# Brian-Acosta/fcc_qp

Measured on NVIDIA B200. Metric: qps_solved_per_sec_batch_65536_cold, higher is better.
Workload: dtype f64

## Files before the change

### fcc_qp_b200/csrc/fccqp_capi.cu

```cuda
#include <cuda_runtime.h>

#include <atomic>
#include <chrono>
#include <cmath>
#include <cstdarg>
#include <cstdio>
#include <cstring>
#include <map>
#include <memory>
#include <mutex>
#include <thread>
#include <string>
#include <vector>

#include "../../include/fccqp.h"
#include "fccqp_kernel.cuh"
#include "fccqp_struct.cuh"
#include "fccqp_warp.cuh"
#include "fccqp_polish.cuh"

namespace {

thread_local std::string g_err;
std::atomic<long long> g_launches{0};
// ... 91 lines not shown
using KernelFn = void (*)(const fccqp::SolveParams);

struct DevSwitches {
  bool no_warp = false;
  bool no_shared = false;
  int full_inverse_at = 0;
  int cta_cap = 0;
#ifdef FCCQP_DEV
  bool profile = false;
#endif
};

const DevSwitches& dev_switches() {
  static const DevSwitches s = [] {
    DevSwitches d;
    d.no_warp = getenv("FCCQP_NO_WARP") != nullptr;
    d.no_shared = getenv("FCCQP_NO_SHARED") != nullptr;
    if (const char* v = getenv("FCCQP_FULL_INVERSE_AT")) d.full_inverse_at = atoi(v) < 1 ? 1 : atoi(v);
    if (const char* v = getenv("FCCQP_CTAS_PER_SM")) d.cta_cap = atoi(v);
#ifdef FCCQP_DEV
    d.profile = getenv("FCCQP_PROFILE") != nullptr;
#endif
    return d;
  }();
  return s;
}

int check_shape(const DeviceCtx& ctx, int n, int m, int nc) {
  const int N = n + m;
  if (N < 1) return fail(FCCQP_E_INVALID, "n + m must be >= 1");
  const fccqp::Layout l(n, m, nc);
  if (l.N8 > 256 || l.bytes() > (size_t)ctx.max_smem_optin)
    return fail(FCCQP_E_UNSUPPORTED,
                "n + m = %d (padded %d) needs %zu B of shared memory per QP (limit %d B, 256 rows): too large "
                "for the shared-memory-resident kernels", N, l.N8, l.bytes(), ctx.max_smem_optin);
  return FCCQP_OK;
}

template <int kThreads, int kMinBlocks>
KernelFn solve_instance(bool shared, bool f32, bool adapt) {
  using fccqp::fccqp_solve_kernel;
  if (shared) return fccqp_solve_kernel<kThreads, kMinBlocks, true, false>;
  if (f32) return adapt ? fccqp_solve_kernel<kThreads, kMinBlocks, false, true, true> : fccqp_solve_kernel<kThreads, kMinBlocks, false, true>;
  return adapt ? fccqp_solve_kernel<kThreads, kMinBlocks, false, false, true> : fccqp_solve_kernel<kThreads, kMinBlocks, false, false>;
}
KernelFn pick_kernel(int threads, bool shared, bool f32, bool adapt) {
  return threads == 128 ? solve_instance<128, 4>(shared, f32, adapt) : solve_instance<256, 2>(shared, f32, adapt);
}

template <int kThreads, int kMinBlocks>
KernelFn struct_instance(bool adapt) {
  return adapt ? fccqp::fccqp_struct_kernel<kThreads, kMinBlocks, true> : fccqp::fccqp_struct_kernel<kThreads, kMinBlocks, false>;
}

bool host_classify(int n, int m, const double* Q, long long q_rs, long long q_cs, const double* A, long long a_rs,
                   long long a_cs, int* nr, int* ndp, int* nd0) {
  std::vector<int> rowcnt(m > 0 ? m : 1, 0), one_row(n, -1);
  std::vector<char> type(n, 0);
  bool ok = true;
  for (int j = 0; j < n; ++j) {
    bool sep = true;
    for (int i = 0; i < n && sep; ++i)
      if (i != j && (Q[i * q_rs + j * q_cs] != 0.0 || Q[j * q_rs + i * q_cs] != 0.0)) sep = false;
    const double qd = Q[j * q_rs + j * q_cs];
    int nnz = 0, kr = 0;
    for (int k = 0; k < m; ++k) if (A[k * a_rs + j * a_cs] != 0.0) { ++nnz; kr = k; }
    if (!sep || !(qd >= 0.0)) type[j] = fccqp::VT_R;
    else if (qd < 1e-200) { type[j] = fccqp::VT_D0; if (nnz == 0) ok = false; }
    else if (nnz <= 1) { type[j] = fccqp::VT_D1; if (nnz == 1) { one_row[j] = kr; ++rowcnt[kr]; } }
    else type[j] = fccqp::VT_DP;
  }
  *nr = *ndp = *nd0 = 0;
  for (int j = 0; j < n; ++j) {
    if (type[j] == fccqp::VT_D1 && one_row[j] >= 0 && rowcnt[one_row[j]] > 1) type[j] = fccqp::VT_DP;
    if (type[j] == fccqp::VT_R) ++*nr; else if (type[j] == fccqp::VT_DP) ++*ndp; else if (type[j] == fccqp::VT_D0) ++*nd0;
  }
  return ok;
}

int geometry(DeviceCtx& ctx, KernelFn fn, int threads, size_t smem, int B, int qps_per_cta, LaunchInfo* li) {
  int c = 0;
  {
    std::lock_guard<std::mutex> lk(ctx.mu);
    const auto key = std::make_pair((const void*)fn, smem);
    auto it = ctx.occupancy.find(key);
    if (it != ctx.occupancy.end()) c = it->second;
    else {
      CUDA_TRY(cudaFuncSetAttribute(fn, cudaFuncAttributeMaxDynamicSharedMemorySize, ctx.max_smem_optin));
      CUDA_TRY(cudaOccupancyMaxActiveBlocksPerMultiprocessor(&c, fn, threads, smem));
      if (c < 1) return fail(FCCQP_E_UNSUPPORTED, "kernel does not fit on an SM (smem %zu B)", smem);
      ctx.occupancy[key] = c;
    }
  }
  const int cap = dev_switches().cta_cap;
  if (cap > 0 && cap < c) c = cap;
  const int need = (B + qps_per_cta - 1) / qps_per_cta;
  *li = {c * ctx.num_sms < need ? c * ctx.num_sms : need, threads, (int)smem, c};
  return FCCQP_OK;
}

struct Scratch {
  static constexpr size_t kWork = 0;
  static constexpr size_t kWork2 = 1;
  static constexpr size_t kListCount = 2;
  static constexpr size_t kProbe = 4;
  static constexpr size_t kLpt = 8;
  static constexpr size_t kHeader = 16;
  unsigned int* w = nullptr;
  size_t B = 0;
  int* list() const { return reinterpret_cast<int*>(w + kHeader); }
  int* order() const { return reinterpret_cast<int*>(w + kHeader + B); }
};

int begin_call(fccqp::SolveParams& p, cudaStream_t stream, bool lpt_hint, long long slots, Scratch* s) {
  const bool lpt = lpt_hint && p.n_iter != nullptr && p.B >= 2 * slots;
  s->B = (size_t)p.B;
  CUDA_TRY(cudaMallocAsync(&s->w, (Scratch::kHeader + (lpt ? 2 : 1) * s->B) * sizeof(unsigned int), stream));
  CUDA_TRY(cudaMemsetAsync(s->w, 0, Scratch::kHeader * sizeof(unsigned int), stream));
  p.work_counter = s->w + Scratch::kWork;
  if (lpt) {
    fccqp::lpt_order_kernel<<<(p.B + 255) / 256, 256, 0, stream>>>(p.n_iter, p.B, p.full_inverse_at, s->order(),
                                                                   s->w + Scratch::kLpt, s->w + Scratch::kLpt + 1);
    CUDA_TRY(cudaGetLastError());
    p.index_list = s->order();
  }
  return FCCQP_OK;
}

int end_call(const Scratch& s, cudaStream_t stream, int launches, const LaunchInfo& li, const StructInfo& si) {
  CUDA_TRY(cudaFreeAsync(s.w, stream));
  g_launches.fetch_add(launches);
  std::lock_guard<std::mutex> lk(g_info_mu);
  g_last_launch = li;
  g_last_struct = si;
  return FCCQP_OK;
}

StructInfo dense_info(const DeviceCtx& ctx, int rows) {
  StructInfo si;
  si.rows = si.rows_dense = rows;
  si.device = ctx.device;
  return si;
}

#ifdef FCCQP_DEV
struct PhaseProfile {
  unsigned long long* d = nullptr;
  int start(cudaStream_t stream, fccqp::SolveParams* p) {
    if (!dev_switches().profile) return FCCQP_OK;
    CUDA_TRY(cudaMalloc(&d, 16 * sizeof(unsigned long long)));
    CUDA_TRY(cudaMemsetAsync(d, 0, 16 * sizeof(unsigned long long), stream));
    p->prof = d;
    return FCCQP_OK;
  }
  int report(cudaStream_t stream, const char* kernel, const char* const (&names)[16], int B, int grid) {
    if (!d) return FCCQP_OK;
    unsigned long long h[16];
    CUDA_TRY(cudaMemcpyAsync(h, d, sizeof(h), cudaMemcpyDeviceToHost, stream));
    CUDA_TRY(cudaStreamSynchronize(stream));
    CUDA_TRY(cudaFree(d));
    const double qps = (double)h[14];
    double tot = 0;
    for (int i = 0; i < 16; ++i) if (names[i]) tot += (double)h[i];
    fprintf(stderr, "[fccqp %s profile] B=%d grid=%d qps=%llu", kernel, B, grid, h[14]);
    if (!names[15]) fprintf(stderr, " iters=%llu", h[15]);
    fprintf(stderr, " cycles/QP=%.0f\n", qps > 0 ? tot / qps : 0.0);
    for (int i = 0; i < 16; ++i)
      if (names[i])
        fprintf(stderr, "   %-14s %10.0f cyc/QP  %5.1f%%\n", names[i], qps > 0 ? (double)h[i] / qps : 0.0,
                tot > 0 ? 100.0 * (double)h[i] / tot : 0.0);
// ... 22 lines not shown
  CUDA_TRY(cudaGetLastError());
  return end_call(s, stream, 1, li, dense_info(ctx, N));
}

int launch_shared(DeviceCtx& ctx, fccqp::SolveParams p, cudaStream_t stream, const Scratch& s) {
  const int threads = p.lay.N8 <= 128 ? 128 : 256;
  KernelFn fn = pick_kernel(threads, true, false, false);
  LaunchInfo li;
  int rc = geometry(ctx, fn, threads, p.lay.bytes(), p.B, 1, &li);
  if (rc) return rc;
  p.shared_mode = 2;
  if (!p.warm) {
    fccqp::SolveParams a = p;
    a.shared_mode = 1;
    a.pending_count = s.w + Scratch::kListCount;
    a.pending_list = s.list();
    fn<<<li.grid, li.block, li.smem, stream>>>(a);
    CUDA_TRY(cudaGetLastError());
    p.count_dev = a.pending_count;
    p.index_list = s.list();
    p.work_counter = s.w + Scratch::kWork2;
  }
  fn<<<li.grid, li.block, li.smem, stream>>>(p);
  CUDA_TRY(cudaGetLastError());
  return end_call(s, stream, p.warm ? 1 : 2, li, dense_info(ctx, p.lay.N8));
}

constexpr int kNotApplicable = 1;

int launch_struct(DeviceCtx& ctx, const fccqp::SolveParams& p, cudaStream_t stream, const Scratch& s, const StructHint& hint,
                  KernelFn general, const LaunchInfo& gli) {
  int caps[3] = {hint.caps[0], hint.caps[1], hint.caps[2]};
  if (hint.mode != FCCQP_STRUCTURE_CAPS) {
    const int ns = p.B < 128 ? p.B : 128;
    int* d_probe = reinterpret_cast<int*>(s.w + Scratch::kProbe);
    if (p.n <= 128 && p.m <= 128) fccqp::fccqp_struct_probe_kernel<128><<<ns, 128, 0, stream>>>(p, ns, d_probe);
    else fccqp::fccqp_struct_probe_kernel<256><<<ns, 256, 0, stream>>>(p, ns, d_probe);
    CUDA_TRY(cudaGetLastError());
    int h[4];
    {
      std::lock_guard<std::mutex> lk(ctx.mu);
      CUDA_TRY(cudaMemcpyAsync(ctx.h_probe, d_probe, sizeof(h), cudaMemcpyDeviceToHost, stream));
      CUDA_TRY(cudaStreamSynchronize(stream));
      memcpy(h, ctx.h_probe, sizeof(h));
    }
    g_launches.fetch_add(1);
    if (h[3] != 0) return kNotApplicable;
    caps[0] = h[0]; caps[1] = h[1]; caps[2] = h[2];
  }
  if (caps[0] < 0 || caps[0] > p.n || caps[1] < 0 || caps[2] < 0 || caps[0] + caps[1] + caps[2] > p.n) return kNotApplicable;
  const fccqp::StructLayout sl(p.n, p.m, p.nc, caps[0], caps[1] + caps[2], caps[2]);
  if (sl.N8c + 8 > p.lay.N8 || sl.bytes() > (size_t)ctx.max_smem_optin) return kNotApplicable;
  const int need = p.n > sl.N8c ? p.n : sl.N8c;
  const bool adapt = p.adapt_k > 0;
  KernelFn fn;
  int threads;
  if (need <= 64) { threads = 64; fn = struct_instance<64, 8>(adapt); }
  else if (need <= 96) { threads = 96; fn = struct_instance<96, 5>(adapt); }
  else if (need <= 128) { threads = 128; fn = struct_instance<128, 4>(adapt); }
  else { threads = 256; fn = struct_instance<256, 2>(adapt); }
  LaunchInfo li;
  int rc = geometry(ctx, fn, threads, sl.bytes(), p.B, 1, &li);
  if (rc) return rc;
  fccqp::SolveParams a = p;
  a.slay = sl;
  a.pending_count = s.w + Scratch::kListCount;
  a.pending_list = s.list();
  const long long neT = sl.n8 >> 3, NBr = sl.nr8c >> 3, mt = sl.mt;
  a.op_stride = (2 * mt * neT + neT * NBr + neT * (neT + 1) / 2) * 64 + 8 * neT;
  CUDA_TRY(cudaMallocAsync(&a.op_scratch, (size_t)li.grid * a.op_stride * sizeof(double), stream));
#ifdef FCCQP_DEV
  PhaseProfile prof;
  if ((rc = prof.start(stream, &a))) return rc;
#endif
  fn<<<li.grid, li.block, li.smem, stream>>>(a);
  CUDA_TRY(cudaGetLastError());
  CUDA_TRY(cudaFreeAsync(a.op_scratch, stream));
#ifdef FCCQP_DEV
  if ((rc = prof.report(stream, "struct", kStructPhases, p.B, li.grid))) return rc;
#endif
  fccqp::SolveParams b = p;
  b.count_dev = a.pending_count;
  b.index_list = s.list();
  b.work_counter = s.w + Scratch::kWork2;
  general<<<gli.grid, gli.block, gli.smem, stream>>>(b);
  CUDA_TRY(cudaGetLastError());
  CUDA_TRY(cudaMemcpyAsync(ctx.h_deferred, a.pending_count, sizeof(unsigned int), cudaMemcpyDeviceToHost, stream));
  StructInfo si;
  si.used = 1; si.nr = caps[0]; si.ndp = caps[1]; si.nd0 = caps[2]; si.rows = sl.N8c; si.rows_dense = p.lay.N8; si.device = ctx.device;
  return end_call(s, stream, 2, li, si);
}

int launch_general(DeviceCtx& ctx, fccqp::SolveParams p, cudaStream_t stream, const Scratch& s, KernelFn fn, const LaunchInfo& li) {
#ifdef FCCQP_DEV
  PhaseProfile prof;
  int rc = prof.start(stream, &p);
  if (rc) return rc;
#endif
  fn<<<li.grid, li.block, li.smem, stream>>>(p);
  CUDA_TRY(cudaGetLastError());
#ifdef FCCQP_DEV
  if ((rc = prof.report(stream, "general", kGeneralPhases, p.B, li.grid))) return rc;
#endif
  return end_call(s, stream, 1, li, dense_info(ctx, p.lay.N8));
}

int launch_solve(DeviceCtx& ctx, fccqp::SolveParams p, cudaStream_t stream, int precision, const StructHint& hint) {
  if (p.B == 0) return FCCQP_OK;
  int rc = check_shape(ctx, p.n, p.m, p.nc);
  if (rc) return rc;
  const DevSwitches& sw = dev_switches();
  const bool f32 = precision != FCCQP_PRECISION_FP64;
  const bool small = p.n + p.m <= 32;
  p.lay = fccqp::Layout(p.n, p.m, p.nc);
  p.full_inverse_at = sw.full_inverse_at ? sw.full_inverse_at : (small ? 8 : 6);
  p.struct_refine = hint.refine;
  if (small && (precision == FCCQP_PRECISION_FP32 || (!f32 && !sw.no_warp)))
    return launch_warp(ctx, p, stream, precision == FCCQP_PRECISION_FP32, hint.lpt);

  const int threads = p.lay.N8 <= 128 ? 128 : 256;
  KernelFn general = pick_kernel(threads, false, f32, p.adapt_k > 0);
  LaunchInfo li;
  Scratch s;
  if ((rc = geometry(ctx, general, threads, p.lay.bytes(), p.B, 1, &li)) ||
      (rc = begin_call(p, stream, hint.lpt, (long long)li.ctas_per_sm * ctx.num_sms, &s)))
    return rc;
  if (!sw.no_shared && !f32 && p.q_bs == 0 && (p.m == 0 || p.a_bs == 0) && p.B >= 4 * li.ctas_per_sm * ctx.num_sms)
    return launch_shared(ctx, p, stream, s);
  if (!f32 && hint.mode != FCCQP_STRUCTURE_DENSE && p.m > 0 &&
      (rc = launch_struct(ctx, p, stream, s, hint, general, li)) != kNotApplicable)
    return rc;
  return launch_general(ctx, p, stream, s, general, li);
}

int check_dims(int n, int m, int nc, int lcs) {
  if (n < 0 || m < 0 || nc < 0) return fail(FCCQP_E_INVALID, "negative dimension");
  if (nc % 3 != 0) return fail(FCCQP_E_INVALID, "nc = %d must be a multiple of 3 (src/fcc_qp.cpp:32)", nc);
  if (lcs < 0 || lcs + nc > n)
    return fail(FCCQP_E_INVALID, "lambda_c_start + nc = %d exceeds num_vars = %d (src/fcc_qp.cpp:33)", lcs + nc, n);
  if (n < 1) return fail(FCCQP_E_INVALID, "num_vars must be >= 1");
  return FCCQP_OK;
}

// ... 754 lines not shown
```

### fcc_qp_b200/csrc/fccqp_kernel.cuh

```cuda
#pragma once
#include <cuda_runtime.h>
#include <stdint.h>

namespace fccqp {

struct Layout {
  int n, m, nc;
  int n8, m8, N8;
  int NB, NBx;
  int NB32, NT;
  int NBT;
  int off_M, off_dinv, off_dneg, off_tbuf, off_ybuf, off_xs, off_lcbar, off_muc, off_mu;
  int off_red, off_int;
  int doubles_total;
  static inline int up2(int v) { return (v + 1) & ~1; }
  Layout() = default;
  Layout(int n_, int m_, int nc_) {
    n = n_; m = m_; nc = nc_;
    n8 = (n + 7) & ~7; m8 = (m + 7) & ~7; N8 = n8 + m8;
    NB = N8 >> 3; NBx = n8 >> 3;
    NB32 = (N8 + 31) >> 5; NT = NB32 * 32;
    NBT = NB * (NB + 1) / 2;
    int o = 0;
    off_M = o;     o += NBT * 64;
// ... 59 lines not shown
    off_muc = o;   o += up2(nc + 2);
    off_mu = o;    o += up2(nc / 3 + 2);
    off_red = o;   o += 4 * 32 + 16;
    off_int = o;
    int io = 8;
    io_vtype = io;  io += n8;
    io_vpos = io;   io += n8;
    io_rlist = io;  io += nr8c + 8;
    io_dplist = io; io += ndp8c + 8;
    io_d0list = io; io += nd08c + 8;
    io_d1var = io;  io += m8 + 8;
    io_rowcnt = io; io += m8 + 8;
    io_wtot = io;   io += 32 * 3;
    io_nzflag = io; io += n8;
    io_colcnt = io; io += n8;
    io_colk = io;   io += n8;
    ints_total = io;
    o += (io + 1) / 2;
    doubles_total = o;
  }
  size_t bytes() const { return (size_t)doubles_total * sizeof(double); }
};

struct SolveParams {
  int B, n, m, nc, lcs;
  int max_iter, warm;
  int shared_mode;
  const int* index_list;
  const unsigned int* count_dev;
  int* pending_list;
  unsigned int* pending_count;
  int full_inverse_at;
  double rho, eps_fcone, eps_bound;
  double alpha;
  int adapt_k;
  const double* Q;   long long q_bs, q_rs, q_cs;
  const double* b;   long long b_bs;
  const double* A;   long long a_bs, a_rs, a_cs;
  const double* beq; long long beq_bs;
  const double* mu;  long long mu_bs;
  const double* lb;  long long lb_bs;
  const double* ub;  long long ub_bs;
  double* x; double* mu_x; double* mu_c;
  int* n_iter; int* status;
  double* res_b; double* res_f; double* bviol; double* fviol;
  unsigned int* work_counter;
  unsigned long long* cycles;
  unsigned long long* prof;
  Layout lay;
  StructLayout slay;
  int struct_refine;
  double* op_scratch;
  long long op_stride;
};

__device__ __forceinline__ double warp_max(double v) {
#pragma unroll
  for (int o = 16; o > 0; o >>= 1) v = fmax(v, __shfl_xor_sync(0xffffffffu, v, o));
  return v;
}
__device__ __forceinline__ double warp_sum(double v) {
#pragma unroll
  for (int o = 16; o > 0; o >>= 1) v += __shfl_xor_sync(0xffffffffu, v, o);
  return v;
}

template <bool kSum>
__device__ __forceinline__ void block_reduce2(double& a, double& b, double* red, int& parity) {
  const int lane = threadIdx.x & 31, warp = threadIdx.x >> 5, nw = blockDim.x >> 5;
  double va = a, vb = b;
#pragma unroll
  for (int o = 16; o > 0; o >>= 1) {
    const double oa = __shfl_xor_sync(0xffffffffu, va, o), ob = __shfl_xor_sync(0xffffffffu, vb, o);
    if (kSum) { va += oa; vb += ob; } else { va = fmax(va, oa); vb = fmax(vb, ob); }
  }
  double* r = red + parity * 64;
  if (lane == 0) { r[warp] = va; r[32 + warp] = vb; }
  __syncthreads();
  double ra = r[0], rb = r[32];
#pragma unroll 1
  for (int w = 1; w < nw; ++w) {
    if (kSum) { ra += r[w]; rb += r[32 + w]; } else { ra = fmax(ra, r[w]); rb = fmax(rb, r[32 + w]); }
  }
  a = ra; b = rb;
  parity ^= 1;
}

constexpr double kPivotRatio = 1e-12;
constexpr double kRegDelta = 1e-10;
constexpr int kRegTries = 4;

__device__ __forceinline__ double fast_rcp(double d) {
  double x;
  asm("rcp.approx.ftz.f64 %0, %1;" : "=d"(x) : "d"(d));
  const double e = fma(-d, x, 1.0);
  const double t = fma(e, e, e);
  return fma(x, t, x);
}

__device__ __forceinline__ void cp_async4(void* smem_dst, const void* gsrc) {
  const unsigned s = (unsigned)__cvta_generic_to_shared(smem_dst);
  asm volatile("cp.async.ca.shared.global [%0], [%1], 4;" ::"r"(s), "l"(gsrc) : "memory");
}
__device__ __forceinline__ void cp_async8(double* smem_dst, const double* gsrc) {
  const unsigned s = (unsigned)__cvta_generic_to_shared(smem_dst);
  asm volatile("cp.async.ca.shared.global [%0], [%1], 8;" ::"r"(s), "l"(gsrc) : "memory");
// ... 1225 lines not shown
```

### fcc_qp_b200/csrc/fccqp_struct.cuh

```cuda
#pragma once
#include "fccqp_kernel.cuh"

namespace fccqp {

enum : int { VT_R = 0, VT_DP = 1, VT_D1 = 2, VT_D0 = 3, VT_NONE = 4 };

struct VarClass {
  int type, pos, krow, nnz;
  double aval, qd;
};

struct StructInts {
  int *vtype, *vpos, *rlist, *dplist, *d0list, *d1var, *rowcnt, *wtot, *nzflag, *colcnt, *colk;
};

__device__ __forceinline__ unsigned smem_u32(const void* p) { return (unsigned)__cvta_generic_to_shared(p); }
__device__ __forceinline__ void cp_async8_s(unsigned smem_dst, const double* gsrc) {
  asm volatile("cp.async.ca.shared.global [%0], [%1], 8;" ::"r"(smem_dst), "l"(gsrc) : "memory");
}
__device__ __forceinline__ void mbar_init(unsigned long long* bar, int count) {
  asm volatile("mbarrier.init.shared::cta.b64 [%0], %1;" ::"r"(smem_u32(bar)), "r"(count) : "memory");
  asm volatile("fence.mbarrier_init.release.cluster;" ::: "memory");
}
__device__ __forceinline__ void bulk_g2s(void* dst, const void* src, unsigned bytes, unsigned long long* bar) {
// ... 720 lines not shown
      if (ib < NBF) s0 += col_dot8(M + tile_off(ib, tb) + colo, colc, flip, tbuf + ib * 8);
      out[t] = xbt + (s0 + s1);
    }
    __syncthreads();
    rx = 0.0; rc = 0.0;
    if (is_x) {
      val = out[ci];
      const double xh = relax ? fma(alpha, val, (1.0 - alpha) * xbar) : val;
      const double xb = clampd(xh + mux, lb, ub);
      xbar = xb;
      const double rr = xh - xb;
      mux += rr;
      rx = fabs(rr);
      if (!in_cone) tbuf[ci] = shift * (xbar - mux);
    }
    if (contact) {
      double x0 = out[c0], x1 = out[c1], x2 = out[c2];
      if (relax) {
        x0 = fma(alpha, x0, (1.0 - alpha) * lcbar[3 * t]);
        x1 = fma(alpha, x1, (1.0 - alpha) * lcbar[3 * t + 1]);
        x2 = fma(alpha, x2, (1.0 - alpha) * lcbar[3 * t + 2]);
      }
      double o0, o1, o2;
      project_cone3(x0 + muc[3 * t], x1 + muc[3 * t + 1], x2 + muc[3 * t + 2], mu_t, o0, o1, o2);
      lcbar[3 * t] = o0; lcbar[3 * t + 1] = o1; lcbar[3 * t + 2] = o2;
      const double r0 = x0 - o0, r1 = x1 - o1, r2 = x2 - o2;
      const double m0 = muc[3 * t] + r0, m1 = muc[3 * t + 1] + r1, m2 = muc[3 * t + 2] + r2;
      muc[3 * t] = m0; muc[3 * t + 1] = m1; muc[3 * t + 2] = m2;
      rc = fmax(fabs(r0), fmax(fabs(r1), fabs(r2)));
      tbuf[c0] = shift * (o0 - m0); tbuf[c1] = shift * (o1 - m1); tbuf[c2] = shift * (o2 - m2);
    }
    if (rx != rx || rc != rc) nan_seen = 1;
    conv = __syncthreads_and((rc < a.eps_fcone) && (rx < a.eps_bound));
    if (conv || iter + 1 == a.iters) break;
  }
  if (is_x) smem[a.xs + t] = val;
  th.xbar = xbar; th.mux = mux; th.x = val; th.rx = rx; th.rc = rc; th.conv = conv; th.nan_seen = nan_seen;
  return iter;
}

#ifdef FCCQP_DEV
#define SPROF(slot)                                                        \
  do {                                                                     \
    if (p.prof && tid == 0) {                                              \
      const long long t_now = clock64();                                   \
      s_prof[slot] += (unsigned long long)(t_now - t_prof);                \
      t_prof = t_now;                                                      \
    }                                                                      \
  } while (0)
#else
#define SPROF(slot) do { } while (0)
#endif

template <int kThreads, int kMinBlocks, bool kAdapt>
__global__ void __launch_bounds__(kThreads, kMinBlocks) fccqp_struct_kernel(const SolveParams p) {
  extern __shared__ __align__(16) double smem[];
  const StructLayout& L = p.slay;
  const int tid = threadIdx.x, lane = tid & 31, warp = tid >> 5;
  constexpr int kWarps = kThreads / 32;
  const int n = p.n, m = p.m, nc = p.nc, lcs = p.lcs;
  const int n8 = L.n8, m8 = L.m8, mt = L.mt, dptc = L.dptc;

  double* const M = smem + L.off_M;
  double* const AP = smem + L.off_AP;
  double* const dinv = smem + L.off_dinv;
  double* const dneg = smem + L.off_dneg;
  double* const vd = smem + L.off_vd;
  double* const hinv = smem + L.off_hinv;
  double* const beqs = smem + L.off_beq;
  double* const qd_s = smem + L.off_qd;
  double* const xs = smem + L.off_xs;
  double* const lcbar = smem + L.off_lcbar;
  double* const muc = smem + L.off_muc;
  double* const vmu = smem + L.off_mu;
  double* const red = smem + L.off_red;
  int* const ibuf = reinterpret_cast<int*>(smem + L.off_int);
  int* const s_work = ibuf;
  StructInts I;
  I.vtype = ibuf + L.io_vtype; I.vpos = ibuf + L.io_vpos; I.rlist = ibuf + L.io_rlist; I.dplist = ibuf + L.io_dplist;
  I.d0list = ibuf + L.io_d0list; I.d1var = ibuf + L.io_d1var; I.rowcnt = ibuf + L.io_rowcnt; I.wtot = ibuf + L.io_wtot;
  I.nzflag = ibuf + L.io_nzflag; I.colcnt = ibuf + L.io_colcnt; I.colk = ibuf + L.io_colk;
  double* const rf = smem + L.off_rf;
  StageCtl sc;
  sc.bar = reinterpret_cast<unsigned long long*>(ibuf + 2);
  sc.phase = 0;
  if (tid == 0) mbar_init(sc.bar, 1);

#ifdef FCCQP_DEV
  unsigned long long* const s_prof = reinterpret_cast<unsigned long long*>(smem + L.off_red + 4 * 32);
  long long t_prof = 0;
  if (p.prof && tid == 0) { for (int i = 0; i < 16; ++i) s_prof[i] = 0; t_prof = clock64(); }
#endif
  int parity = 0;
  const int t = tid;
  const bool is_x = t < n;
  const bool in_cone = is_x && t >= lcs && t < lcs + nc;
  const int fr = lane >> 2, fq = lane & 3;
  const int fragC = (fr << 3) + (((fq ^ (fr >> 1)) & 3) << 1);
  const long long q_slow = p.q_cs <= p.q_rs ? p.q_rs : p.q_cs;
  const long long q_fast = p.q_cs <= p.q_rs ? p.q_cs : p.q_rs;
  const bool q_dense = q_fast == 1 && q_slow == n;
  const bool a_dense = (p.a_cs == 1 && p.a_rs == n) || (p.a_rs == 1 && p.a_cs == m);

  int w_next = 0;
  if (tid == 0) {
    w_next = (int)atomicAdd(p.work_counter, 1u);
    if (p.index_list && w_next < p.B) w_next = p.index_list[w_next];
  }
  for (;;) {
    __syncthreads();
    if (tid == 0) {
      s_work[0] = w_next;
      if (w_next < p.B) {
        w_next = (int)atomicAdd(p.work_counter, 1u);
        if (p.index_list && w_next < p.B) w_next = p.index_list[w_next];
      }
    }
    __syncthreads();
    const int qp = s_work[0];
    if (qp >= p.B) break;
    const double* Qg = p.Q + (size_t)qp * p.q_bs;
    const double* Ag = p.A + (size_t)qp * p.a_bs;
    SPROF(0);

    double v_b = 0.0, v_lb = 0.0, v_ub = 0.0, v_mux = 0.0, v_xbar = 0.0, v_x = 0.0;
    int finite_bounds = 0;
    if (is_x) {
      v_b = p.b[(size_t)qp * p.b_bs + t];
      v_lb = p.lb[(size_t)qp * p.lb_bs + t];
      v_ub = p.ub[(size_t)qp * p.ub_bs + t];
      if (p.warm) { v_x = p.x[(size_t)qp * n + t]; v_mux = p.mu_x[(size_t)qp * n + t]; }
    }
    if (t < m) beqs[t] = p.beq[(size_t)qp * p.beq_bs + t];
    if (t < nc / 3) vmu[t] = p.mu[(size_t)qp * p.mu_bs + t];
    if (t < nc) muc[t] = p.warm ? p.mu_c[(size_t)qp * nc + t] : 0.0;
    for (int e = t; e < L.ndp8c + 8; e += kThreads) { vd[e] = 0.0; hinv[e] = 0.0; }

    const long long t_start = clock64();
    unsigned long long fact_cycles = 0;
    int status_flag = 0;
    int n_iter = 0;
    double res_x = 0.0, res_c = 0.0;

    VarClass vc;
    StructQP S;
    const bool q_vec = q_fast == 1 && (n & 1) == 0 && (q_slow & 1) == 0 && (reinterpret_cast<uintptr_t>(Qg) & 15) == 0;
    const bool a_vec = p.a_cs == 1 && (n & 1) == 0 && (p.a_rs & 1) == 0 && (reinterpret_cast<uintptr_t>(Ag) & 15) == 0;
    sc.q_bulk = q_vec && q_slow == n;
    sc.a_bulk = a_vec && p.a_rs == n;
    bool defer = struct_classify<kThreads>(n, m, n8, m8, Qg, q_slow, q_fast, q_vec, Ag, p.a_rs, p.a_cs, a_vec, M, L.stage_cap, sc,
                                           qd_s, rf, I, L.nr8c, L.ndp8c, L.nd08c, vc, S.nr, S.ndp, S.nd0) != 0;
    SPROF(1);
    if (tid == 0 && w_next < p.B) {
      if (q_dense) l2_prefetch(p.Q + (size_t)w_next * p.q_bs, (size_t)n * n * sizeof(double));
      if (a_dense) l2_prefetch(p.A + (size_t)w_next * p.a_bs, (size_t)m * n * sizeof(double));
    }
    S.nr8 = (S.nr + 7) & ~7;
    const int NBr = S.nr8 >> 3;
    const int yrow = t - S.nr8;
    if (is_x && (!isinf(v_lb) || !isinf(v_ub))) finite_bounds = 1;
    if (t < n8) xs[t] = v_x;
    const bool eqc = (nc == 0) && (__syncthreads_or(finite_bounds) == 0);
    const bool presolve = eqc || !p.warm;

    for (int pass = presolve ? 0 : 1; pass < 2 && !defer; ++pass) {
      if (pass == 1 && eqc) break;
      if (pass == 1) {
        v_xbar = v_x;
        if (in_cone) lcbar[t - lcs] = v_x;
        __syncthreads();
        n_iter = p.max_iter;
      }
      const int iters = pass == 0 ? 1 : p.max_iter;
      double shift = pass == 0 ? 0.0 : p.rho;
      VarClass ve = vc;
      StructQP Se = S;
      if (pass == 1 && S.nd0 > 0) {
        if (vc.type == VT_D0) { ve.type = VT_DP; ve.pos = S.ndp + (vc.pos - S.nr8 - m8); }
        Se.ndp = S.ndp + S.nd0;
        Se.nd0 = 0;
      }
      Se.dpt = (Se.ndp + 7) >> 3;
      Se.N8 = S.nr8 + m8 + ((Se.nd0 + 7) & ~7);
      Se.NB = Se.N8 >> 3;
      Se.NB32 = (Se.N8 + 31) >> 5;
      double hi = (ve.type == VT_DP || ve.type == VT_D1) ? 1.0 / (ve.qd + shift) : 0.0;
      bool factored = false;
      bool full_inverse = false;
      bool full_op = false;
      int ci = -1, NBF = 0, NF = 0;
      double v_xbase = 0.0;

#pragma unroll 1
      for (int iter = 0; iter < iters; ++iter) {
        double val = v_x;
        if (!(pass == 1 && iter == 0 && presolve)) {
          if (!factored) {
            factored = true;
            const long long t_f0 = clock64();
            {
              const int nbt = (Se.NB * (Se.NB + 1)) >> 1;
              const double2 z2 = make_double2(0.0, 0.0);
              for (int e = t; e < nbt * 32; e += kThreads) st2(M + 2 * e, z2);
              for (int e = t; e < mt * dptc * 32; e += kThreads) st2(AP + 2 * e, z2);
            }
            if (is_x) { I.vtype[t] = ve.type; I.vpos[t] = ve.pos; }
            __syncthreads();
            {
              constexpr int kCol = kThreads / 32;
              const unsigned mS = smem_u32(M), apS = smem_u32(AP);
              int ckind[kCol], cps[kCol], chf[kCol];
              unsigned cof[kCol];
#pragma unroll
              for (int u = 0; u < kCol; ++u) {
                const int j = lane + 32 * u;
                const int ty = j < n ? I.vtype[j] : VT_NONE;
                const int ps = j < n ? I.vpos[j] : 0;
                ckind[u] = ty == VT_R ? 0 : (ty == VT_DP ? 1 : (ty == VT_D0 ? 2 : 3));
                cps[u] = ps;
                chf[u] = (ps & 7) >> 1;
                cof[u] = ty == VT_D0 ? mS + (unsigned)tile_off(ps >> 3, 0) * 8u + ((ps & 7) << 6)
                                     : (unsigned)(((ps >> 3) << 9) + ((ps & 1) << 3));
              }
#pragma unroll 1
              for (int a = warp; a < S.nr; a += kWarps) {
                const double* qrow = Qg + (long long)I.rlist[a] * q_slow;
                const unsigned rowS = mS + (unsigned)tile_off(a >> 3, 0) * 8u + ((a & 7) << 6);
                const int rh = (a & 7) >> 1;
#pragma unroll
                for (int u = 0; u < kCol; ++u)
                  if (ckind[u] == 0 && cps[u] <= a)
                    cp_async8_s(rowS + cof[u] + (((chf[u] ^ rh) & 3) << 4), qrow + (long long)(lane + 32 * u) * q_fast);
              }
              if (p.a_cs == 1 || p.a_rs != 1) {
#pragma unroll 1
                for (int k = warp; k < m; k += kWarps) {
                  const double* arow = Ag + (long long)k * p.a_rs;
                  const int yr = S.nr8 + k, rh = (k & 7) >> 1;
                  const unsigned rowM = mS + (unsigned)tile_off(yr >> 3, 0) * 8u + ((k & 7) << 6);
                  const unsigned rowP = apS + (unsigned)((k >> 3) * dptc) * 512u + ((k & 7) << 6);
                  const unsigned colT = (unsigned)(((yr >> 3) << 9) + ((yr & 1) << 3));
#pragma unroll
                  for (int u = 0; u < kCol; ++u) {
                    const int kd = ckind[u];
                    const unsigned base = kd == 0 ? rowM : (kd == 1 ? rowP : colT);
                    if (kd < 3) cp_async8_s(base + cof[u] + (((chf[u] ^ rh) & 3) << 4), arow + (long long)(lane + 32 * u) * p.a_cs);
                  }
                }
              } else {
// ... 12 lines not shown
              }
            }
            if (t < Se.N8) {
              const bool pad = (t >= S.nr && t < S.nr8) || (yrow >= m && yrow < m8) || (t >= S.nr8 + m8 + Se.nd0);
              if (pad) M[mat_off(t, t)] = 1.0;
            }
            if (ve.type == VT_D0) M[mat_off(ve.pos, ve.pos)] = ve.qd + shift;
            if (ve.type == VT_DP) hinv[ve.pos] = hi;
            SPROF(2);
            cp_async_wait_all();
            __syncthreads();
            SPROF(3);
            if (t < S.nr && shift != 0.0) M[mat_off(t, t)] += shift;
            {
              const int ntile = (mt * (mt + 1)) >> 1;
#pragma unroll 1
              for (int w = warp; w < ntile; w += kWarps) {
                int Ic = 0;
                while (((Ic + 1) * (Ic + 2)) >> 1 <= w) ++Ic;
                const int Jc = w - ((Ic * (Ic + 1)) >> 1);
                double2 ca = make_double2(0.0, 0.0), cb = make_double2(0.0, 0.0);
                const double* ai = AP + (size_t)(Ic * dptc) * 64 + fragC;
                const double* aj = AP + (size_t)(Jc * dptc) * 64 + fragC;
#pragma unroll 1
                for (int kt = 0; kt < Se.dpt; ++kt) {
                  const double2 a = ld2(ai + 64 * kt), b = ld2(aj + 64 * kt), h = ld2(hinv + 8 * kt + 2 * fq);
                  dmma(ca.x, ca.y, a.x * h.x, b.x);
                  dmma(cb.x, cb.y, a.y * h.y, b.y);
                }
                st2(M + tile_off(NBr + Ic, NBr + Jc) + fragC, make_double2(-(ca.x + cb.x), -(ca.y + cb.y)));
              }
            }
            __syncthreads();
            if (ve.type == VT_D1 && ve.nnz == 1) M[mat_off(S.nr8 + ve.krow, S.nr8 + ve.krow)] -= ve.aval * ve.aval * hi;
            if (yrow >= m && yrow < m8) M[mat_off(t, t)] = 1.0;
            __syncthreads();
            SPROF(4);
            factor_tiles<kThreads>(M, dinv, dneg, Se.NB, Se.NB32);
            SPROF(5);
            fact_cycles += (unsigned long long)(clock64() - t_f0);
            {
              bool badp = false;
              const bool neg = yrow >= 0 && yrow < m;
              const double dn = t < Se.N8 ? dneg[t] : 0.0;
              if (t < Se.N8) badp = !isfinite(dn) || (neg ? !(dn > 0.0) : !(dn < 0.0));
              double pc = neg ? fabs(dn) : 0.0, pu = 0.0;
              block_reduce2<false>(pc, pu, red, parity);
              if (neg && fabs(dn) < kPivotRatio * pc) badp = true;
              if (__syncthreads_or(badp)) { defer = true; break; }
            }
          }

          const double w = (pass == 1 && is_x) ? (in_cone ? (lcbar[t - lcs] - muc[t - lcs]) : (v_xbar - v_mux)) : 0.0;
          const bool make_op = pass == 1 && !full_inverse && iter >= p.full_inverse_at;
#pragma unroll 1
          for (int rep = make_op ? 0 : 1; rep < 2; ++rep) {
            const bool base_solve = rep == 0;
            if (!base_solve && full_op) {
              val = full_op_apply(M, smem + L.off_tbuf, smem + L.off_ybuf, smem + L.off_sred, ci, shift * w, NBF, NF);
              break;
            }
            const bool op = !base_solve && full_inverse;
            double r = 0.0;
            if (is_x) r = (base_solve || pass == 0) ? -v_b : (op ? shift * w : -(v_b - shift * w));
#ifdef FCCQP_DEV
            const double res = struct_xsolve<kThreads>(p, L, smem, I, Se, ve, Qg, Ag, q_slow, q_fast, r, hi, shift, op, op,
                                                       pass == 0 && p.struct_refine != 0, q_vec && a_vec, s_prof, t_prof);
#else
            const double res = struct_xsolve<kThreads>(p, L, smem, I, Se, ve, Qg, Ag, q_slow, q_fast, r, hi, shift, op, op,
                                                       pass == 0 && p.struct_refine != 0, q_vec && a_vec);
#endif
            if (base_solve) {
              v_xbase = res;
              __syncthreads();
              SPROF(12);
              complete_inverse<kThreads>(M, Se.NB);
              SPROF(13);
              form_g<kThreads>(M, dinv, Se.NB, Se.NB, Se.NB);
              SPROF(15);
              full_inverse = true;
              if (p.op_stride > 0) {
                FullOpDims fd;
                fd.NBr = NBr; fd.mt = mt; fd.dptc = dptc; fd.dpt = Se.dpt;
                fd.ne = n - S.nr; fd.neT = (fd.ne + 7) >> 3; fd.NBF = NBr + fd.neT; fd.NF = fd.NBF * 8;
                if (fd.NF <= kThreads && fd.NF <= L.NTc && tile_off(fd.NBF, 0) <= L.stage_cap) {
                  const bool is_d1 = is_x && ve.type == VT_D1;
                  const unsigned b1 = __ballot_sync(0xffffffffu, is_d1);
                  if (lane == 0) I.wtot[warp] = __popc(b1);
                  __syncthreads();
                  int o1 = 0;
  #pragma unroll
                  for (int w2 = 0; w2 < kWarps; ++w2) if (w2 < warp) o1 += I.wtot[w2];
                  int epos = -1;
                  if (is_x && ve.type == VT_DP) epos = ve.pos;
                  else if (is_d1) epos = Se.ndp + o1 + __popc(b1 & ((1u << lane) - 1u));
                  ci = is_x ? (ve.type == VT_R ? ve.pos : S.nr8 + epos) : -1;
                  NBF = fd.NBF; NF = fd.NF;
                  build_full_op<kThreads>(M, AP, hinv, p.op_scratch + (size_t)blockIdx.x * p.op_stride, fd, is_x ? ve.type : VT_NONE,
                                          epos, ve.krow, ve.nnz, ve.aval, hi);
                  SPROF(10);
                  double* const tb2 = smem + L.off_tbuf;
                  double* const xb2 = smem + L.off_ybuf;
                  if (t < NF) { tb2[t] = 0.0; xb2[t] = 0.0; }
                  __syncthreads();
                  if (ci >= 0) xb2[ci] = v_xbase;
                  full_op = true;
                }
              }
            } else {
              val = op ? v_xbase + res : res;
            }
          }
        }
        SPROF(12);

        if (pass == 0) {
          v_x = val;
          if (t < n8) xs[t] = is_x ? val : 0.0;
          __syncthreads();
          continue;
        }

        if (is_x) { xs[t] = val; v_x = val; }
        __syncthreads();
        double rx = 0.0, rc = 0.0, dz = 0.0;
        const bool relax = p.alpha != 1.0;
        if (is_x) {
          const double xh = relax ? fma(p.alpha, val, (1.0 - p.alpha) * v_xbar) : val;
          const double xb = clampd(xh + v_mux, v_lb, v_ub);
          if (kAdapt) dz = fabs(xb - v_xbar);
          v_xbar = xb;
          const double rr = xh - xb;
          v_mux += rr;
          rx = fabs(rr);
        }
        if (t < nc / 3) {
          const int o = lcs + 3 * t;
          double x0 = xs[o], x1 = xs[o + 1], x2 = xs[o + 2];
          if (relax) {
            x0 = fma(p.alpha, x0, (1.0 - p.alpha) * lcbar[3 * t]);
            x1 = fma(p.alpha, x1, (1.0 - p.alpha) * lcbar[3 * t + 1]);
            x2 = fma(p.alpha, x2, (1.0 - p.alpha) * lcbar[3 * t + 2]);
          }
          double o0, o1, o2;
          project_cone3(x0 + muc[3 * t], x1 + muc[3 * t + 1], x2 + muc[3 * t + 2], vmu[t], o0, o1, o2);
          if (kAdapt)
            dz = fmax(dz, fmax(fabs(o0 - lcbar[3 * t]), fmax(fabs(o1 - lcbar[3 * t + 1]), fabs(o2 - lcbar[3 * t + 2]))));
          lcbar[3 * t] = o0; lcbar[3 * t + 1] = o1; lcbar[3 * t + 2] = o2;
          const double r0 = x0 - o0, r1 = x1 - o1, r2 = x2 - o2;
          muc[3 * t] += r0; muc[3 * t + 1] += r1; muc[3 * t + 2] += r2;
          rc = fmax(fabs(r0), fmax(fabs(r1), fabs(r2)));
        }
        if (rx != rx || rc != rc) status_flag = 2;
        const int conv = __syncthreads_and((rc < p.eps_fcone) && (rx < p.eps_bound));
        if (conv || iter + 1 == iters) {
          block_reduce2<false>(rx, rc, red, parity);
          res_x = rx; res_c = rc;
          if (conv) { n_iter = iter; SPROF(8); break; }
        } else if (!kAdapt && kThreads > 64 && full_op) {
          OpLoopArgs oa;
          oa.M = (int)(M - smem); oa.tbuf = L.off_tbuf; oa.xb = L.off_ybuf; oa.out = L.off_sred; oa.xs = (int)(xs - smem);
          oa.lcbar = L.off_lcbar; oa.muc = L.off_muc; oa.vmu = L.off_mu;
          oa.ints = L.off_int; oa.cidx = L.io_colk;
          oa.NBF = NBF; oa.NF = NF; oa.nc = nc; oa.lcs = lcs; oa.iter0 = iter + 1; oa.iters = iters;
          oa.shift = shift; oa.alpha = p.alpha; oa.eps_fcone = p.eps_fcone; oa.eps_bound = p.eps_bound;
          OpLoopThread th;
          th.xbar = v_xbar; th.mux = v_mux; th.lb = v_lb; th.ub = v_ub; th.x = v_x; th.ci = ci;
          const int it_end = full_op_loop(oa, th, is_x, in_cone);
          v_xbar = th.xbar; v_mux = th.mux;
          if (is_x) v_x = th.x;
          if (th.nan_seen) status_flag = 2;
          rx = th.rx; rc = th.rc;
          block_reduce2<false>(rx, rc, red, parity);
          res_x = rx; res_c = rc;
          if (th.conv) n_iter = it_end;
          SPROF(8);
          break;
        } else if (kAdapt && p.adapt_k > 0 && (iter + 1) % p.adapt_k == 0) {
          double rp = fmax(rx, rc), rd = dz;
          block_reduce2<false>(rp, rd, red, parity);
          rd *= shift;
          double ratio = sqrt(rp / (rd > 1e-300 ? rd : 1e-300));
          ratio = fmin(fmax(ratio, 0.1), 10.0);
          if (ratio > 5.0 || ratio < 0.2) {
            const double rho_new = fmin(fmax(shift * ratio, 1e-9), 1e9);
            const double sc = shift / rho_new;
            v_mux *= sc;
            if (t < nc / 3) { muc[3 * t] *= sc; muc[3 * t + 1] *= sc; muc[3 * t + 2] *= sc; }
            shift = rho_new;
            hi = (ve.type == VT_DP || ve.type == VT_D1) ? 1.0 / (ve.qd + shift) : 0.0;
            factored = false; full_inverse = false; full_op = false;
            __syncthreads();
          }
        }
        SPROF(8);
      }
    }

    if (defer) {
      if (tid == 0) p.pending_list[atomicAdd(p.pending_count, 1u)] = qp;
      continue;
    }
    __syncthreads();
    double bv = 0.0, fv = 0.0;
    int bad = 0;
    if (is_x) {
      const double d = v_x - clampd(v_x, v_lb, v_ub);
      bv = d * d;
      if (!isfinite(v_x)) bad = 1;
    }
    if (tid < nc / 3) {
      const int o = lcs + 3 * tid;
      const double rr = sqrt(xs[o] * xs[o] + xs[o + 1] * xs[o + 1]) - vmu[tid] * xs[o + 2];
      fv = rr > 0.0 ? rr : 0.0;
    }
    block_reduce2<true>(bv, fv, red, parity);
    bad = __syncthreads_or(bad | (status_flag == 2));
    if (is_x) {
      p.x[(size_t)qp * n + t] = v_x;
      if (p.mu_x) p.mu_x[(size_t)qp * n + t] = v_mux;
    }
    if (p.mu_c && t < nc) p.mu_c[(size_t)qp * nc + t] = muc[t];
    if (tid == 0) {
      if (p.n_iter) p.n_iter[qp] = n_iter;
      if (p.status) p.status[qp] = bad ? 2 : (n_iter == p.max_iter ? 1 : 0);
      if (p.res_b) p.res_b[qp] = res_x;
      if (p.res_f) p.res_f[qp] = res_c;
      if (p.bviol) p.bviol[qp] = sqrt(bv);
      if (p.fviol) p.fviol[qp] = fv;
      if (p.cycles) {
        atomicAdd(p.cycles, fact_cycles);
        atomicAdd(p.cycles + 1, (unsigned long long)(clock64() - t_start));
      }
    }
    SPROF(9);
#ifdef FCCQP_DEV
    if (p.prof && tid == 0) s_prof[14] += 1;
#endif
  }
#ifdef FCCQP_DEV
  if (p.prof && tid == 0)
    for (int i = 0; i < 16; ++i) atomicAdd(p.prof + i, s_prof[i]);
#endif
}

}
```

Before: 11.99 million.

## Split cold structured solve into a light first-stage kernel plus resume kernel

For cold batches large enough relative to resident CTAs, launches a first-stage struct kernel that runs the presolve pass and the first iteration without building the full operator. QPs that converge there are finished, and the rest are written to a resume list with x saved. A second launch of the full kernel then processes only the resume list, starting from pass 1. The aim is to keep heavy operator-building and its scratch, along with their occupancy cost, off QPs that converge early, and to balance load across the batch. The cost is an extra launch, global round-trips of x for surviving QPs, and the factorization being redone in the resume kernel.

```diff
diff --git a/fcc_qp_b200/csrc/fccqp_capi.cu b/fcc_qp_b200/csrc/fccqp_capi.cu
--- a/fcc_qp_b200/csrc/fccqp_capi.cu
+++ b/fcc_qp_b200/csrc/fccqp_capi.cu
@@ -167,6 +167,12 @@
 KernelFn struct_instance(bool adapt) {
   return adapt ? fccqp::fccqp_struct_kernel<kThreads, kMinBlocks, true> : fccqp::fccqp_struct_kernel<kThreads, kMinBlocks, false>;
 }
+template <int kThreads, int kMinBlocks>
+KernelFn struct_first_instance(bool refine) {
+  using fccqp::fccqp_struct_kernel;
+  return refine ? fccqp_struct_kernel<kThreads, kMinBlocks, false, fccqp::kStructFirstRefine>
+                : fccqp_struct_kernel<kThreads, kMinBlocks, false, fccqp::kStructFirst>;
+}
 
 bool host_classify(int n, int m, const double* Q, long long q_rs, long long q_cs, const double* A, long long a_rs,
                    long long a_cs, int* nr, int* ndp, int* nd0) {
@@ -220,17 +226,20 @@
   static constexpr size_t kListCount = 2;
   static constexpr size_t kProbe = 4;
   static constexpr size_t kLpt = 8;
+  static constexpr size_t kWork3 = 10;
+  static constexpr size_t kResumeCount = 11;
   static constexpr size_t kHeader = 16;
   unsigned int* w = nullptr;
   size_t B = 0;
   int* list() const { return reinterpret_cast<int*>(w + kHeader); }
-  int* order() const { return reinterpret_cast<int*>(w + kHeader + B); }
+  int* resume_list() const { return reinterpret_cast<int*>(w + kHeader + B); }
+  int* order() const { return reinterpret_cast<int*>(w + kHeader + 2 * B); }
 };
 
 int begin_call(fccqp::SolveParams& p, cudaStream_t stream, bool lpt_hint, long long slots, Scratch* s) {
   const bool lpt = lpt_hint && p.n_iter != nullptr && p.B >= 2 * slots;
   s->B = (size_t)p.B;
-  CUDA_TRY(cudaMallocAsync(&s->w, (Scratch::kHeader + (lpt ? 2 : 1) * s->B) * sizeof(unsigned int), stream));
+  CUDA_TRY(cudaMallocAsync(&s->w, (Scratch::kHeader + (lpt ? 3 : 2) * s->B) * sizeof(unsigned int), stream));
   CUDA_TRY(cudaMemsetAsync(s->w, 0, Scratch::kHeader * sizeof(unsigned int), stream));
   p.work_counter = s->w + Scratch::kWork;
   if (lpt) {
@@ -359,20 +368,44 @@
   const fccqp::StructLayout sl(p.n, p.m, p.nc, caps[0], caps[1] + caps[2], caps[2]);
   if (sl.N8c + 8 > p.lay.N8 || sl.bytes() > (size_t)ctx.max_smem_optin) return kNotApplicable;
   const int need = p.n > sl.N8c ? p.n : sl.N8c;
-  const bool adapt = p.adapt_k > 0;
+  const bool adapt = p.adapt_k > 0, refine = p.struct_refine != 0;
+  int threads;
+  KernelFn first;
+  if (need <= 64) { threads = 64; first = struct_first_instance<64, 8>(refine); }
+  else if (need <= 96) { threads = 96; first = struct_first_instance<96, 5>(refine); }
+  else if (need <= 128) { threads = 128; first = struct_first_instance<128, 4>(refine); }
+  else { threads = 256; first = struct_first_instance<256, 2>(refine); }
+  LaunchInfo li, fli;
+  int rc = geometry(ctx, first, threads, sl.bytes(), p.B, 1, &fli);
+  if (rc) return rc;
+  const bool split = !p.warm && p.B >= 8LL * fli.ctas_per_sm * ctx.num_sms;
   KernelFn fn;
-  int threads;
-  if (need <= 64) { threads = 64; fn = struct_instance<64, 8>(adapt); }
-  else if (need <= 96) { threads = 96; fn = struct_instance<96, 5>(adapt); }
-  else if (need <= 128) { threads = 128; fn = struct_instance<128, 4>(adapt); }
-  else { threads = 256; fn = struct_instance<256, 2>(adapt); }
-  LaunchInfo li;
-  int rc = geometry(ctx, fn, threads, sl.bytes(), p.B, 1, &li);
-  if (rc) return rc;
+  if (threads == 64) fn = struct_instance<64, 8>(adapt);
+  else if (threads == 96) fn = struct_instance<96, 5>(adapt);
+  else if (threads == 128) fn = struct_instance<128, 4>(adapt);
+  else fn = struct_instance<256, 2>(adapt);
+  if ((rc = geometry(ctx, fn, threads, sl.bytes(), p.B, 1, &li))) return rc;
   fccqp::SolveParams a = p;
   a.slay = sl;
   a.pending_count = s.w + Scratch::kListCount;
   a.pending_list = s.list();
+  if (split) {
+    fccqp::SolveParams f = a;
+    f.resume_list = s.resume_list();
+    f.resume_count = s.w + Scratch::kResumeCount;
+#ifdef FCCQP_DEV
+    PhaseProfile prof;
+    if ((rc = prof.start(stream, &f))) return rc;
+#endif
+    first<<<fli.grid, fli.block, fli.smem, stream>>>(f);
+    CUDA_TRY(cudaGetLastError());
+#ifdef FCCQP_DEV
+    if ((rc = prof.report(stream, "struct first stage", kStructPhases, p.B, fli.grid))) return rc;
+#endif
+    a.count_dev = f.resume_count;
+    a.index_list = f.resume_list;
+    a.work_counter = s.w + Scratch::kWork3;
+  }
   const long long neT = sl.n8 >> 3, NBr = sl.nr8c >> 3, mt = sl.mt;
   a.op_stride = (2 * mt * neT + neT * NBr + neT * (neT + 1) / 2) * 64 + 8 * neT;
   CUDA_TRY(cudaMallocAsync(&a.op_scratch, (size_t)li.grid * a.op_stride * sizeof(double), stream));
@@ -384,7 +417,7 @@
   CUDA_TRY(cudaGetLastError());
   CUDA_TRY(cudaFreeAsync(a.op_scratch, stream));
 #ifdef FCCQP_DEV
-  if ((rc = prof.report(stream, "struct", kStructPhases, p.B, li.grid))) return rc;
+  if ((rc = prof.report(stream, split ? "struct resume" : "struct", kStructPhases, p.B, li.grid))) return rc;
 #endif
   fccqp::SolveParams b = p;
   b.count_dev = a.pending_count;
@@ -395,7 +428,7 @@
   CUDA_TRY(cudaMemcpyAsync(ctx.h_deferred, a.pending_count, sizeof(unsigned int), cudaMemcpyDeviceToHost, stream));
   StructInfo si;
   si.used = 1; si.nr = caps[0]; si.ndp = caps[1]; si.nd0 = caps[2]; si.rows = sl.N8c; si.rows_dense = p.lay.N8; si.device = ctx.device;
-  return end_call(s, stream, 2, li, si);
+  return end_call(s, stream, split ? 3 : 2, split ? fli : li, si);
 }
 
 int launch_general(DeviceCtx& ctx, fccqp::SolveParams p, cudaStream_t stream, const Scratch& s, KernelFn fn, const LaunchInfo& li) {
diff --git a/fcc_qp_b200/csrc/fccqp_kernel.cuh b/fcc_qp_b200/csrc/fccqp_kernel.cuh
--- a/fcc_qp_b200/csrc/fccqp_kernel.cuh
+++ b/fcc_qp_b200/csrc/fccqp_kernel.cuh
@@ -135,6 +135,8 @@
   int struct_refine;
   double* op_scratch;
   long long op_stride;
+  int* resume_list;
+  unsigned int* resume_count;
 };
 
 __device__ __forceinline__ double warp_max(double v) {
diff --git a/fcc_qp_b200/csrc/fccqp_struct.cuh b/fcc_qp_b200/csrc/fccqp_struct.cuh
--- a/fcc_qp_b200/csrc/fccqp_struct.cuh
+++ b/fcc_qp_b200/csrc/fccqp_struct.cuh
@@ -796,8 +796,12 @@
 #define SPROF(slot) do { } while (0)
 #endif
 
-template <int kThreads, int kMinBlocks, bool kAdapt>
+enum : int { kStructFull = 0, kStructFirst = 1, kStructFirstRefine = 2 };
+
+template <int kThreads, int kMinBlocks, bool kAdapt, int kStage = kStructFull>
 __global__ void __launch_bounds__(kThreads, kMinBlocks) fccqp_struct_kernel(const SolveParams p) {
+  constexpr bool kFirst = kStage != kStructFull;
+  static_assert(!(kFirst && kAdapt), "the first stage stops before adaptive rho can act");
   extern __shared__ __align__(16) double smem[];
   const StructLayout& L = p.slay;
   const int tid = threadIdx.x, lane = tid & 31, warp = tid >> 5;
@@ -849,6 +853,7 @@
   int w_next = 0;
   if (tid == 0) {
     w_next = (int)atomicAdd(p.work_counter, 1u);
+    if (!kFirst && p.count_dev && w_next >= (int)*p.count_dev) w_next = p.B;
     if (p.index_list && w_next < p.B) w_next = p.index_list[w_next];
   }
   for (;;) {
@@ -857,12 +862,14 @@
       s_work[0] = w_next;
       if (w_next < p.B) {
         w_next = (int)atomicAdd(p.work_counter, 1u);
+        if (!kFirst && p.count_dev && w_next >= (int)*p.count_dev) w_next = p.B;
         if (p.index_list && w_next < p.B) w_next = p.index_list[w_next];
       }
     }
     __syncthreads();
     const int qp = s_work[0];
     if (qp >= p.B) break;
+    const bool resume = !kFirst && p.count_dev != nullptr;
     const double* Qg = p.Q + (size_t)qp * p.q_bs;
     const double* Ag = p.A + (size_t)qp * p.a_bs;
     SPROF(0);
@@ -873,7 +880,8 @@
       v_b = p.b[(size_t)qp * p.b_bs + t];
       v_lb = p.lb[(size_t)qp * p.lb_bs + t];
       v_ub = p.ub[(size_t)qp * p.ub_bs + t];
-      if (p.warm) { v_x = p.x[(size_t)qp * n + t]; v_mux = p.mu_x[(size_t)qp * n + t]; }
+      if (p.warm || resume) v_x = p.x[(size_t)qp * n + t];
+      if (p.warm) v_mux = p.mu_x[(size_t)qp * n + t];
     }
     if (t < m) beqs[t] = p.beq[(size_t)qp * p.beq_bs + t];
     if (t < nc / 3) vmu[t] = p.mu[(size_t)qp * p.mu_bs + t];
@@ -907,7 +915,8 @@
     const bool eqc = (nc == 0) && (__syncthreads_or(finite_bounds) == 0);
     const bool presolve = eqc || !p.warm;
 
-    for (int pass = presolve ? 0 : 1; pass < 2 && !defer; ++pass) {
+    bool survive = false;
+    for (int pass = (presolve && !resume) ? 0 : 1; pass < 2 && !defer; ++pass) {
       if (pass == 1 && eqc) break;
       if (pass == 1) {
         v_xbar = v_x;
@@ -938,7 +947,7 @@
 #pragma unroll 1
       for (int iter = 0; iter < iters; ++iter) {
         double val = v_x;
-        if (!(pass == 1 && iter == 0 && presolve)) {
+        if (kFirst ? pass == 0 : !(pass == 1 && iter == 0 && presolve)) {
           if (!factored) {
             factored = true;
             const long long t_f0 = clock64();
@@ -1057,25 +1066,28 @@
           }
 
           const double w = (pass == 1 && is_x) ? (in_cone ? (lcbar[t - lcs] - muc[t - lcs]) : (v_xbar - v_mux)) : 0.0;
-          const bool make_op = pass == 1 && !full_inverse && iter >= p.full_inverse_at;
+          const bool make_op = !kFirst && pass == 1 && !full_inverse && iter >= p.full_inverse_at;
+          const bool refine = kFirst ? kStage == kStructFirstRefine : (pass == 0 && p.struct_refine != 0);
 #pragma unroll 1
           for (int rep = make_op ? 0 : 1; rep < 2; ++rep) {
             const bool base_solve = rep == 0;
-            if (!base_solve && full_op) {
+            if (!kFirst && !base_solve && full_op) {
               val = full_op_apply(M, smem + L.off_tbuf, smem + L.off_ybuf, smem + L.off_sred, ci, shift * w, NBF, NF);
               break;
             }
-            const bool op = !base_solve && full_inverse;
+            const bool op = !kFirst && !base_solve && full_inverse;
             double r = 0.0;
             if (is_x) r = (base_solve || pass == 0) ? -v_b : (op ? shift * w : -(v_b - shift * w));
 #ifdef FCCQP_DEV
             const double res = struct_xsolve<kThreads>(p, L, smem, I, Se, ve, Qg, Ag, q_slow, q_fast, r, hi, shift, op, op,
-                                                       pass == 0 && p.struct_refine != 0, q_vec && a_vec, s_prof, t_prof);
+                                                       refine, q_vec && a_vec, s_prof, t_prof);
 #else
             const double res = struct_xsolve<kThreads>(p, L, smem, I, Se, ve, Qg, Ag, q_slow, q_fast, r, hi, shift, op, op,
-                                                       pass == 0 && p.struct_refine != 0, q_vec && a_vec);
+                                                       refine, q_vec && a_vec);
 #endif
-            if (base_solve) {
+            if constexpr (kFirst) {
+              val = res;
+            } else if (base_solve) {
               v_xbase = res;
               __syncthreads();
               SPROF(12);
@@ -1162,6 +1174,9 @@
           block_reduce2<false>(rx, rc, red, parity);
           res_x = rx; res_c = rc;
           if (conv) { n_iter = iter; SPROF(8); break; }
+        } else if (kFirst) {
+          survive = true;
+          break;
         } else if (!kAdapt && kThreads > 64 && full_op) {
           OpLoopArgs oa;
           oa.M = (int)(M - smem); oa.tbuf = L.off_tbuf; oa.xb = L.off_ybuf; oa.out = L.off_sred; oa.xs = (int)(xs - smem);
@@ -1206,6 +1221,11 @@
       if (tid == 0) p.pending_list[atomicAdd(p.pending_count, 1u)] = qp;
       continue;
     }
+    if (kFirst && survive) {
+      if (is_x) p.x[(size_t)qp * n + t] = v_x;
+      if (tid == 0) p.resume_list[atomicAdd(p.resume_count, 1u)] = qp;
+      continue;
+    }
     __syncthreads();
     double bv = 0.0, fv = 0.0;
     int bad = 0;
```

Measured after the change: 13.40 million, median of 6. 11.8% higher.
